# ISAE-PNX/SaDVIO

Hardware: AMD Instinct MI355X
Metric: BA iterations/sec (ms/solve in ms_per_solve), 20-KF/8k-landmark window (higher is better)
Workload: dtype f64; 1 GPU; synthetic 20 KF x 8000 landmarks x 40000 reprojection factors (pixel), GN 10 iters (LM step attempts, early exits disabled); windows_per_gpu=1, parallelism=single window, n_kf=20, n_lmk=8000, n_obs=40000, reduced_dim=114

## Files before the change

sadvio_amd/csrc/ba_handle.h:

```cpp
#pragma once
#include <hip/hip_runtime.h>
#include <dlfcn.h>

#include <algorithm>
#include <chrono>
#include <cmath>
#include <cstdio>
#include <cstdlib>
#include <cstring>
#include <map>
#include <string>
#include <vector>

#include "../../include/sadvio_ba.h"
#include "kernels.h"
#include "layout_plan.h"
#include "dense_chol.h"
#include "marg_kernels.h"
#include "lm_kernels.h"
#include "long_kernels.h"
#include "viinit_kernels.h"
#include "nofov_kernels.h"

using namespace sadvio;
// ... 199 lines not shown
    std::vector<int> h_pairs, h_ptr, h_lmk, h_last;
    int csr_win = -1;
    int n_kf_lmk = 0;
};

struct EnvCfg {
    int debug = 0;
    int lm = -1, pf_wg = -1;
    int tile_rounds = 0, lm_subs = 0, band_c = 0;
    int cov_batch_lds = 1, cov_batch_scratch_mb = 1024;
    int cov_band = -1;
    int cov_sqrt = -1;
    int cov_cross_stage = -1;
    int long_min_env = 0;
    double jacobi_tol = 1e-14;
    bool marg_pivoted = false, marg_unpivoted = false, pchol_strict = false, no_lpt = false, no_pre = false, no_fork = false, no_bcr = false, imu_items = false, contig_tiles = false, c16_old_tail = false;
    void read() {
        auto on = [](const char* k) { return getenv(k) != nullptr; };
        auto num = [](const char* k, int unset) { const char* e = getenv(k); return e ? atoi(e) : unset; };
        debug = num("SADVIO_DEBUG", 0); lm = num("SADVIO_LM", -1); pf_wg = num("SADVIO_PF_WG", -1);
        tile_rounds = num("SADVIO_TILE_ROUNDS", 0); lm_subs = num("SADVIO_LM_SUBS", 0); band_c = num("SADVIO_BAND_C", 0);
        cov_batch_lds = num("SADVIO_COV_BATCH_LDS", 1); cov_batch_scratch_mb = num("SADVIO_COV_BATCH_SCRATCH_MB", 1024);
        cov_band = num("SADVIO_COV_BAND", -1); cov_sqrt = num("SADVIO_COV_SQRT", -1);
        cov_cross_stage = num("SADVIO_COV_CROSS_STAGE", -1);
        long_min_env = num("SADVIO_LONG_MIN", 0);
        if (long_min_env < 2 || long_min_env > MAX_LMK_OBS + 1) long_min_env = 0;
        if (const char* e = getenv("SADVIO_JACOBI_TOL")) jacobi_tol = atof(e);
        marg_pivoted = on("SADVIO_MARG_PIVOTED"); marg_unpivoted = on("SADVIO_MARG_UNPIVOTED"); pchol_strict = on("SADVIO_PCHOL_STRICT");
        no_lpt = on("SADVIO_NO_LPT"); no_pre = on("SADVIO_NO_PRE"); no_fork = on("SADVIO_NO_FORK");
        no_bcr = on("SADVIO_NO_BCR");
        contig_tiles = on("SADVIO_CONTIG_TILES");
        c16_old_tail = on("SADVIO_C16_OLD_TAIL");
        imu_items = on("SADVIO_IMU_ITEMS");
    }
};

struct LongCfg {
    int min = 0;
    bool priors = false;
    bool cov = false;
    bool batch = false;
    bool from_create(unsigned reserved, int long_min_env, std::string& err) {
        static const struct { unsigned flag; const char* name; const char* reason; } needs[] = {
            {SADVIO_CFG_LONG_TRACK_PRIORS, "SADVIO_CFG_LONG_TRACK_PRIORS", "to carry a prior on"},
            {SADVIO_CFG_LONG_TRACK_COVARIANCE, "SADVIO_CFG_LONG_TRACK_COVARIANCE", "to form a covariance of"},
            {SADVIO_CFG_LONG_TRACK_BATCH, "SADVIO_CFG_LONG_TRACK_BATCH", "for a batch call to serve"}};
        for (const auto& n : needs)
// ... 68 lines not shown
    DevBuf<unsigned char> d_lmk_const;
    DevBuf<int> d_lmk_ob, d_lmk_oe, d_obs_kf, d_obs_cam, d_tile_kf, d_tile_row, d_tile_lmk;
    DevBuf<int> d_long_rec, d_long_kf, d_long_slot;
    DevBuf<int> d_pre_lane, d_pre_kf;
    bool pre_dirty = false;
    DevBuf<int> d_rank_col; DevBuf<double> d_rank_x;
    DevBuf<unsigned char> d_obs_slot, d_obs_lslot;
    DevBuf<int> d_chunk_ob, d_chunk_lm, d_tile_perm;
    DevBuf<int> d_jac_ints;
    DevBuf<double> d_jac_dbl;
    DevBuf<double> d_lm_hg, d_lm_dt, d_lm_sacc;
    DevBuf<int> d_lm_sub;
    int hidden_eig_count = 0;
    int marg_stats[4] = {0, 0, 0, 0};
    DevBuf<double> d_ptab;
    DevBuf<double> d_obs_meas;
    DevBuf<PriorDev> d_priors;
    DevBuf<double> d_prior_lin;
    DevBuf<ImuDev> d_imus;
    DevBuf<double> d_imu_scratch;
    DevBuf<double> d_S, d_gred, d_gfull, d_hdiag, d_delta, d_s_pose;
    DevBuf<LmState> d_states;
    DevBuf<double> d_trace;
    DevBuf<long long> d_tstart;
    DevBuf<IterAcc> d_acc;
    DevBuf<FinalRec> d_final;
    FinalRec* h_final = nullptr;
    double* h_deltas = nullptr; size_t h_deltas_cap = 0; bool deltas_cached = false;
    size_t h_final_n = 0;
    std::vector<FinalRec> fin;
// ... 77 lines not shown
```

sadvio_amd/csrc/kernels.h:

```cpp
#pragma once
#include "ba_types.h"
#include "device_math.h"
#include "chol16.h"

namespace sadvio {

struct DevPtrs {
    const WinDev* win;
    const Tile* tiles;
    const double* kf_T0;
    const int* kf_fidx;
    double* xp; double* xv; double* xba; double* xbg;
    long long xp_stride, xv_stride, xl_stride;
    const double* kf_vel; const double* kf_ba; const double* kf_bg;
    const double* cam_K; const double* cam_T; const double* cam_isig;
    const double* lmk_p; double* xl; double* s_lmk;
    const unsigned char* lmk_const;
    const int* lmk_ob; const int* lmk_oe;
    const int* obs_kf; const int* obs_cam; const double* obs_meas;
    const unsigned char* obs_slot;
    const int* tile_kf;
    const int* tile_lmk;
    const int* tile_row;
    const int4* pre_lane;
// ... 36 lines not shown
    double* lm_dt;
    long long lm_hg_stride, lm_dt_stride;
    const int* lm_sub;
    int lm_sub_per_item;
    int lm_ksub;
    double* lm_sacc;
    const LineDev* lines;
    const LineObsDev* lobs;
    double* xline;
    double* line_scratch;
    long long xline_stride;
    long long n_xp, n_xv, n_xl;
    int n_tiles;
    int state_stride;
    int n_win;
    long long* t_start;
    double* trace;
    long long* dbg_ts;
    int debug;
    int c16_old_tail;
    SolveOpts o;
};

#ifdef SADVIO_KERNEL_TS
#define SADVIO_TS(slot_, idx_) do { if ((P.debug & 4096) && blockIdx.x == 0 && threadIdx.x == 0 && slot == (slot_)) P.dbg_ts[idx_] = wall_clock64(); } while (0)
#define SADVIO_TS_PTR(cond_) ((cond_) ? P.dbg_ts : nullptr)
constexpr int DBG_WG_MAX = 1024, DBG_WG_BASE = 128, DBG_SLOTS = DBG_WG_BASE + 4 * DBG_WG_MAX;
#define SADVIO_WG_TS(slot_, which_) do { if ((P.debug & 4096) && blockIdx.x < DBG_WG_MAX && threadIdx.x == 0 && slot == (slot_)) { \
        P.dbg_ts[DBG_WG_BASE + 4 * blockIdx.x + (which_)] = wall_clock64(); \
        if ((which_) == 0) P.dbg_ts[DBG_WG_BASE + 4 * blockIdx.x + 3] = 0; \
        if ((which_) == 0) P.dbg_ts[DBG_WG_BASE + 4 * blockIdx.x + 2] = ((long long)__builtin_amdgcn_s_getreg(20 | (31 << 11)) << 32) | (unsigned)__builtin_amdgcn_s_getreg(4 | (31 << 11)); } } while (0)
#else
#define SADVIO_TS(slot_, idx_) do { } while (0)
#define SADVIO_TS_PTR(cond_) nullptr
#define SADVIO_WG_TS(slot_, which_) do { } while (0)
constexpr int DBG_SLOTS = 128;
// ... 350 lines not shown
        const int lane0 = tid * 8, wv = lane0 >> 6, ln = lane0 & 63;
        const int G = T.G, lpw = 64 / G, grp = ln / G, q0 = ln - grp * G, nl = T.n_lmk;
        const bool valid = wv * lpw + grp < nl;
        const int gl = nl > 0 ? tile_landmark(T, tile_lmk, valid ? wv * lpw + grp : 0) : T.lmk0;
        const int ob = nl > 0 ? lmk_ob[gl] : 0, nobs = (valid && nl > 0) ? lmk_oe[gl] - ob : 0;
        pre_lane[(long long)blockIdx.x * (BUILD_THREADS / 8) + tid] = make_int4(gl, ob, nobs | (valid ? 1 << 16 : 0), q0);
    }
    if (tid < PRE_KF) {
        int2 e = make_int2(-1, -1);
        if (tid < T.n_kf) { e.x = tile_kf[T.kf_off + tid]; e.y = kf_fidx[e.x]; }
        pre_kf[(long long)blockIdx.x * PRE_KF + tid] = e;
    }
}

template <bool COST_ONLY> __device__ __forceinline__ void pose_factor_eval(const DevPtrs& P, int slot, int idx, int ln);
template <int FACTOR, bool RARE, bool IMU>
__global__ __launch_bounds__(BUILD_THREADS, IMU ? 1 : 2) void k_build(DevPtrs P, int slot, int max_tile_kf, int strip_doubles, int Rp) {
    extern __shared__ __attribute__((aligned(16))) char smem[];
    if (IMU && (int)blockIdx.x >= P.n_tiles) {
        pose_factor_eval<false>(P, slot, (int)blockIdx.x - P.n_tiles, threadIdx.x);
        return;
    }
    const Tile T = P.tiles[blockIdx.x];
    const int tid = threadIdx.x, wv = tid >> 6, ln = tid & 63;
    int4 pl = make_int4(0, -1, 0, 0);
    int2 pk = make_int2(-1, -1);
    if (P.pre_lane) {
        pl = P.pre_lane[(long long)blockIdx.x * (BUILD_THREADS / 8) + (tid >> 3)];
        pk = P.pre_kf[(long long)blockIdx.x * PRE_KF + tid / POSE_TAB];
    }
    SADVIO_TS(3, 32);
    SADVIO_WG_TS(3, 0);
    __shared__ double s_part[BUILD_WAVES * 4];
    double* poseTab = (double*)smem;
    double* camTab = poseTab + (size_t)max_tile_kf * POSE_TAB;
    int* rowTab = (int*)(camTab + MAX_WIN_CAM * 17);
    double* stage = (double*)(smem + tile_tables_bytes(max_tile_kf));
// ... 19 lines not shown
            }
        } else {
            const TileAcc* ta = P.tacc + (long long)((slot - 1) & 1) * P.n_tiles + t0;
            double v[4][4];
#pragma unroll
            for (int u = 0; u < 4; u++) {
                const int t = tid + u * BUILD_THREADS;
                const bool in = t < nt;
                const TileAcc* e = ta + (in ? t : 0);
                v[u][0] = in ? e->cand_cost : 0.0; v[u][1] = in ? e->mcc : 0.0; v[u][2] = in ? e->step_norm2 : 0.0; v[u][3] = in ? e->cand_norm2 : 0.0;
            }
            pc = (v[0][0] + v[1][0]) + (v[2][0] + v[3][0]); pm = (v[0][1] + v[1][1]) + (v[2][1] + v[3][1]);
            psn = (v[0][2] + v[1][2]) + (v[2][2] + v[3][2]); pcn = (v[0][3] + v[1][3]) + (v[2][3] + v[3][3]);
        }
    };
    if (P.n_win == 1) decision_inputs(0, 0, P.n_tiles);
    else decision_inputs(T.w, T.win_tile0, T.win_ntiles);
    bool first_valid;
    int gl_first, pre_ob, pre_oe, pre_o;
    static_assert(MAX_LMK_OBS <= 0xff, "a first-round packet carries the landmark's observation count in 8 bits");
    if (P.pre_lane) {
        first_valid = (pl.z >> 16) & 1; gl_first = pl.x; pre_ob = pl.y; pre_oe = pl.y + (pl.z & 0xff);
        pre_o = (pl.w + (tid & 7) < (pl.z & 0xff)) ? pl.y + pl.w + (tid & 7) : -1;
    } else {
        first_valid = wv * lpw + grp < nl;
        gl_first = tile_landmark(T, P.tile_lmk, first_valid ? wv * lpw + grp : 0);
        pre_ob = P.lmk_ob[gl_first]; pre_oe = P.lmk_oe[gl_first];
        pre_o = (first_valid && q < pre_oe - pre_ob) ? pre_ob + q : -1;
    }
    const int pre_lcode = P.lmk_const ? P.lmk_const[gl_first] : 0;
    double pre_p[3], pre_x0[3], pre_x1[3];
#pragma unroll
    for (int i = 0; i < 3; i++) {
        pre_p[i] = P.lmk_p[3 * (long long)gl_first + i];
        pre_x0[i] = P.xl[3 * (long long)gl_first + i];
        pre_x1[i] = P.xl[P.xl_stride + 3 * (long long)gl_first + i];
    }
    double pre_s[3] = {1.0, 1.0, 1.0};
    if (slot != 0) {
#pragma unroll
        for (int i = 0; i < 3; i++) pre_s[i] = P.s_lmk[3 * (long long)gl_first + i];
    }
    double pre_t0 = 0.0, pre_t1 = 0.0;
    if (P.pre_lane) {
        if (pk.x >= 0) {
            const long long src = (long long)pk.x * POSE_TAB + (tid - (tid / POSE_TAB) * POSE_TAB);
            pre_t0 = P.ptab[src]; pre_t1 = P.ptab[P.ptab_stride + src];
        }
    } else if (tid < T.n_kf * POSE_TAB) {
        const int k = tid / POSE_TAB, e = tid - k * POSE_TAB;
        const long long src = (long long)P.tile_kf[T.kf_off + k] * POSE_TAB + e;
        pre_t0 = P.ptab[src]; pre_t1 = P.ptab[P.ptab_stride + src];
    }
    for (int i = tid; i < T.n_cam * 17; i += blockDim.x) {
        const int c = i / 17, e = i - 17 * c;
        const int gc = T.cam_base + c;
        camTab[i] = e < 4 ? P.cam_K[4 * (long long)gc + e] : (e < 16 ? P.cam_T[12 * (long long)gc + e - 4] : P.cam_isig[gc]);
    }
    for (int i = tid; i < T.n_kf; i += blockDim.x) rowTab[i] = P.tile_row[T.kf_off + i];
    ObsPre pre_obs;
    pre_obs.slot = 0; pre_obs.craw = 0; pre_obs.m[0] = pre_obs.m[1] = pre_obs.m[2] = 0.0;
    if (pre_o >= 0) pre_obs = obs_prefetch<FACTOR>(P, pre_o);
    if (own_decision) {
        pc = wave_sum(pc); pm = wave_sum(pm); psn = wave_sum(psn); pcn = wave_sum(pcn);
        if (ln == 0) { s_part[wv * 4] = pc; s_part[wv * 4 + 1] = pm; s_part[wv * 4 + 2] = psn; s_part[wv * 4 + 3] = pcn; }
        __syncthreads();
        a.cand_cost += (s_part[0] + s_part[4]) + (s_part[8] + s_part[12]); a.mcc += (s_part[1] + s_part[5]) + (s_part[9] + s_part[13]);
// ... 1 lines not shown
        st = lm_decide(prev, a, P.o);
        __syncthreads();
        if (T.first_of_window && tid == 0) { P.states[(long long)T.w * P.state_stride + slot] = st; trace_write(P, T.w, slot - 1, prev, a, st); }
    }
    if (st.done) return;
    SADVIO_TS(3, 33);
    double* Stile = stage + BUILD_WAVES * strip_doubles;
    const int Nt = 6 * T.n_free;
    const int tri_n = Nt * (Nt + 1) / 2;
    double* gT = Stile + tri_n;
    double* gfT = gT + Nt;
    double* hdT = gfT + Nt;
    const bool lds_mode = T.lds_mode != 0;
    if (tid < T.n_kf * POSE_TAB) poseTab[tid] = st.cur ? pre_t1 : pre_t0;
    {
        const double* src = P.ptab + (long long)st.cur * P.ptab_stride;
        for (int i = tid + blockDim.x; i < T.n_kf * POSE_TAB; i += blockDim.x) {
            const int k = i / POSE_TAB, e = i - k * POSE_TAB;
            poseTab[i] = src[(long long)P.tile_kf[T.kf_off + k] * POSE_TAB + e];
        }
    }
    if (lds_mode) {
        const int nz = tri_n + 3 * Nt;
        for (int i = tid; i < nz; i += blockDim.x) Stile[i] = 0.0;
    }
    __syncthreads();

    SADVIO_TS(3, 34);
    double* Sg = P.S + T.S_off;
    double* gredg = P.gred + T.red_off;
    double* gfullg = P.gfull + T.red_off;
// ... 18 lines not shown
        if (!first && slot != 0) {
#pragma unroll
            for (int i = 0; i < 3; i++) sc[i] = P.s_lmk[3 * (long long)gl + i];
        }
        ObsLin L;
        L.valid = q < nobs;
        L.row = -1; L.slot = 0; L.counted = false;
        if (L.valid) {
            double pw[3];
            ObsPre obq;
            if (first) {
#pragma unroll
                for (int i = 0; i < 3; i++) pw[i] = pre_p[i] + (st.cur ? pre_x1[i] : pre_x0[i]);
                obq = pre_obs;
            } else {
#pragma unroll
                for (int i = 0; i < 3; i++) pw[i] = P.lmk_p[3 * (long long)gl + i] + xl[3 * (long long)gl + i];
                obq = obs_prefetch<FACTOR>(P, ob + q);
            }
            lane_linearize<FACTOR, RARE>(P, poseTab, camTab, rowTab, T.cam_base, obq, pw, lfree, lcode != 1, L);
            const double c = L.rho;
            if (L.counted) cost_part += c;
            else { fixed_part += c; L.r[0] = 0.0; L.r[1] = 0.0; }
        } else {
            L.r[0] = L.r[1] = 0.0;
#pragma unroll
            for (int i = 0; i < 12; i++) L.Jp[i] = 0.0;
#pragma unroll
            for (int i = 0; i < 6; i++) L.Jl[i] = 0.0;
        }
    SADVIO_TS(3, 35);
        double Mi[6], g[3];
// ... 184 lines not shown
                    const int row = 16 * tr + lk + 4 * rg;
                    if (row < Nt && col <= row) atomic_add_f64(&Stile[tri(row, col)], -accs[pp][rg]);
                }
            }
        }
    }
    SADVIO_TS(3, 40);
    const double c = wave_sum(cost_part), f = wave_sum(fixed_part), gm = wave_max(gmax_part);
    if (ln == 0) { s_part[wv * 4] = c; s_part[wv * 4 + 1] = f; s_part[wv * 4 + 2] = gm; }
    __syncthreads();
    if (tid == 0) {
        double cs = 0.0, fs = 0.0, gs = 0.0;
        for (int k = 0; k < BUILD_WAVES; k++) { cs += s_part[k * 4]; fs += s_part[k * 4 + 1]; gs = fmax(gs, s_part[k * 4 + 2]); }
        TileAcc* ta = P.tacc + (long long)(slot & 1) * P.n_tiles + blockIdx.x;
        ta->lin_cost = cs; ta->fixed_cost = fs; ta->gmax = gs;
    }
    SADVIO_TS(3, 41);
    if (lds_mode) {
        int* growTab = (int*)stage;
        for (int k = tid; k < T.n_kf; k += blockDim.x) {
            const int r = rowTab[k];
            if (r >= 0) {
                const int fi = P.kf_fidx[P.tile_kf[T.kf_off + k]];
#pragma unroll
                for (int i = 0; i < 6; i++) growTab[r + i] = fi * dpf + i;
            }
        }
        __syncthreads();
        if (T.ld) {
            for (int row = wv; row < Nt; row += BUILD_WAVES) {
// ... 1561 lines not shown
}

__device__ __forceinline__ void init_tables_item(const DevPtrs& P, int g, int n_kf_tot) {
    if (g < P.n_prior_tot) {
        const PriorDev pr = P.priors[g];
        double d6[6] = {0.0, 0.0, 0.0, 0.0, 0.0, 0.0};
        prior_lin_record(P.kf_T0 + 12 * (long long)pr.kf, pr.T_prior, pr.inf, d6, P.prior_lin + (long long)g * PRIOR_LIN);
    }
    if (g >= n_kf_tot) return;
    double d6[6], tab[POSE_TAB];
    for (int i = 0; i < 6; i++) d6[i] = 0.0;
    pose_table_entry(P.kf_T0 + 12 * (long long)g, d6, tab);
    for (int i = 0; i < POSE_TAB; i++) P.ptab[(long long)g * POSE_TAB + i] = tab[i];
}

__global__ void k_decide(DevPtrs P, int slot, int final) {
    const int w = blockIdx.x, ln = threadIdx.x;
    __shared__ double s4[4];
    const WinDev W = P.win[w];
    LmState f;
    const bool already = final && P.decide_kernel;
    if (!already) {
        if (P.lm_sacc) {
            __shared__ double sq[16 * 4];
            const long long n = (long long)(W.tile_end - W.tile_begin) * P.lm_ksub;
            const double* sa = P.lm_sacc + ((long long)(slot & 1) * P.n_tiles + W.tile_begin) * P.lm_ksub * 4;
            double c = 0.0, m = 0.0, sn = 0.0, cn = 0.0;
            for (long long t = ln; t < n; t += blockDim.x) { c += sa[4 * t]; m += sa[4 * t + 1]; sn += sa[4 * t + 2]; cn += sa[4 * t + 3]; }
            c = wave_sum(c); m = wave_sum(m); sn = wave_sum(sn); cn = wave_sum(cn);
            if ((ln & 63) == 0) { double* q = sq + 4 * (ln >> 6); q[0] = c; q[1] = m; q[2] = sn; q[3] = cn; }
// ... 663 lines not shown
```

sadvio_amd/csrc/layout_driver.h:

```cpp
#pragma once
#include "ba_handle.h"

namespace {

__global__ void k_dense_prior_prepare(const double* J, double* Jt, int nf, int n) {
    const long long idx = (long long)blockIdx.x * blockDim.x + threadIdx.x;
    if (idx < (long long)nf * n) {
        const int i = (int)(idx / n), a = (int)(idx - (long long)i * n);
        Jt[(size_t)a * nf + i] = J[idx];
    }
}

__global__ void k_sym_from_lower(const double* __restrict__ A, int n, double* __restrict__ H) {
    const long long idx = (long long)blockIdx.x * blockDim.x + threadIdx.x;
    if (idx >= (long long)n * n) return;
    const int i = (int)(idx / n), j = (int)(idx - (long long)i * n);
    H[idx] = i >= j ? A[idx] : A[(size_t)j * n + i];
}

LayoutIn layout_inputs(sadvio_ba_handle* h) {
    LayoutIn in;
    in.src = &h->src; in.sparse_per_win = &h->sparse_per_win; in.dprior_per_win = &h->dprior_per_win; in.lines_per_win = &h->lines_per_win;
    in.prior_valid = h->prior.valid; in.prior_serial = h->prior.serial; in.prior_n_full = h->prior.n_full; in.prior_n = h->prior.n;
    in.world = h->world; in.has_coll = h->coll_fn != nullptr;
// ... 89 lines not shown
        wins[w].d.imu_end = (int)h->imus.size();
    }
    HIP_TRY(h->d_imus.alloc(h->imus.size()));
    HIP_TRY(h->d_imu_scratch.alloc(2 * h->imus.size() * (size_t)IMU_ROW));
    if (!h->imus.empty())
        h->up.add(h->d_imus.p, h->imus.data(), h->imus.size() * sizeof(ImuDev));
    std::vector<WinDev> wd(wins.size());
    for (size_t w = 0; w < wins.size(); w++) wd[w] = wins[w].d;
    h->up.add(h->d_win.p, wd.data(), wd.size() * sizeof(WinDev));
    HIP_TRY(h->up.flush(h->stream));
    if (h->plan.pre_ok && h->pre_dirty) {
        hipLaunchKernelGGL(k_pre_packets, dim3((unsigned)h->plan.tiles.size()), dim3(BUILD_THREADS), 0, h->stream, h->d_tiles.p, h->d_lmk_ob.p, h->d_lmk_oe.p, h->d_tile_kf.p,
                           h->d_tile_lmk.p, h->d_kf_fidx.p, (int4*)h->d_pre_lane.p, (int2*)h->d_pre_kf.p);
        h->pre_dirty = false;
    }
    return SADVIO_OK;
}

int layout_build(sadvio_ba_handle* h) {
    const bool dbg_t = (h->env.debug & 8192) != 0;
    auto t_start = std::chrono::steady_clock::now();
    auto lap = [&](const char* what) { if (dbg_t) { auto t = std::chrono::steady_clock::now(); fprintf(stderr, "[sadvio dbg] build_layout %-14s %.3f ms\n", what, std::chrono::duration<double, std::milli>(t - t_start).count()); t_start = t; } };
    HIP_TRY(hipSetDevice(h->device));
    h->uploaded = false; h->solved = false;
    h->up.reset();
    LayoutPlan& P = h->plan;
    int rc = layout_plan(layout_inputs(h), P, h->err, lap);
    if (rc != SADVIO_OK) return rc;
    const size_t kf_b = P.n_kf_tot, lmk_b = std::max(P.n_lmk_tot, 1), n_tiles = P.tiles.size();
    if (h->env.debug) {
// ... 7 lines not shown
        fprintf(stderr, "\n");
    }
    if (P.want_lm) {
        HIP_TRY(h->d_lm_hg.alloc(2 * (size_t)LM_HG * lmk_b));
        const size_t n_rec = std::max<size_t>(n_tiles, 1) * P.lm_ksub;
        HIP_TRY(h->d_lm_dt.alloc(2 * (size_t)LM_DT * n_rec));
        HIP_TRY(h->d_lm_sacc.alloc(2 * 4 * n_rec));
        HIP_TRY(hipMemsetAsync(h->d_lm_sacc.p, 0, sizeof(double) * 2 * 4 * n_rec, h->stream));
        HIP_TRY(hipMemsetAsync(h->d_lm_dt.p, 0, sizeof(double) * 2 * (size_t)LM_DT * n_rec, h->stream));
    }
    HIP_TRY(h->d_chunk_ob.alloc(P.chunk_ob.size())); HIP_TRY(h->d_chunk_lm.alloc(P.chunk_lm.size())); HIP_TRY(h->d_obs_lslot.alloc(P.obs_lslot.size()));
    HIP_TRY(h->d_tile_perm.alloc(std::max<size_t>(P.perm.size(), 1))); HIP_TRY(h->d_lm_sub.alloc(std::max<size_t>(P.sub.size(), 2)));
    HIP_TRY(h->d_win.alloc(P.wins.size())); HIP_TRY(h->d_tacc.alloc(2 * n_tiles));
    HIP_TRY(h->d_tile_kf.alloc(P.tile_kf.size())); HIP_TRY(h->d_tile_row.alloc(P.tile_row.size())); HIP_TRY(h->d_tile_lmk.alloc(P.tile_lmk.size()));
    HIP_TRY(h->d_obs_slot.alloc(P.obs_slot.size())); HIP_TRY(h->d_ptab.alloc(2 * (size_t)POSE_TAB * kf_b));
    HIP_TRY(h->d_kf_T0.alloc(P.kf_T0.size())); HIP_TRY(h->d_kf_fidx.alloc(P.kf_fidx.size()));
    HIP_TRY(h->d_xp.alloc(2 * 6 * kf_b)); HIP_TRY(h->d_xv.alloc(2 * 3 * kf_b));
    HIP_TRY(h->d_xba.alloc(2 * 3 * kf_b)); HIP_TRY(h->d_xbg.alloc(2 * 3 * kf_b));
    HIP_TRY(h->d_kf_vel.alloc(P.kf_vel.size())); HIP_TRY(h->d_kf_ba.alloc(P.kf_ba.size())); HIP_TRY(h->d_kf_bg.alloc(P.kf_bg.size()));
    HIP_TRY(h->d_cam_K.alloc(P.cam_K.size())); HIP_TRY(h->d_cam_T.alloc(P.cam_T.size())); HIP_TRY(h->d_cam_isig.alloc(P.cam_isig.size()));
    HIP_TRY(h->d_lmk_p.alloc(P.lmk_p.size())); HIP_TRY(h->d_xl.alloc(2 * 3 * lmk_b));
    HIP_TRY(h->d_s_lmk.alloc(3 * lmk_b));
    HIP_TRY(h->d_lmk_ob.alloc(P.lmk_ob.size())); HIP_TRY(h->d_lmk_oe.alloc(P.lmk_oe.size()));
    HIP_TRY(h->d_obs_kf.alloc(P.obs_kf.size())); HIP_TRY(h->d_obs_cam.alloc(P.obs_cam.size())); HIP_TRY(h->d_obs_meas.alloc(P.obs_meas.size()));
    queue_table(h, h->d_chunk_ob, P.chunk_ob); queue_table(h, h->d_chunk_lm, P.chunk_lm); queue_table(h, h->d_obs_lslot, P.obs_lslot);
    queue_table(h, h->d_tile_perm, P.perm); queue_table(h, h->d_lm_sub, P.sub);
    queue_table(h, h->d_kf_T0, P.kf_T0); queue_table(h, h->d_kf_fidx, P.kf_fidx); queue_table(h, h->d_kf_vel, P.kf_vel);
    queue_table(h, h->d_kf_ba, P.kf_ba); queue_table(h, h->d_kf_bg, P.kf_bg); queue_table(h, h->d_cam_K, P.cam_K); queue_table(h, h->d_cam_T, P.cam_T);
    queue_table(h, h->d_cam_isig, P.cam_isig); queue_table(h, h->d_lmk_p, P.lmk_p);
    queue_table(h, h->d_lmk_ob, P.lmk_ob); queue_table(h, h->d_lmk_oe, P.lmk_oe); queue_table(h, h->d_obs_kf, P.obs_kf);
// ... 25 lines not shown
```

sadvio_amd/csrc/solve_driver.h:

```cpp
#pragma once
#include <cstddef>
#include <type_traits>

#include "ba_handle.h"
#include "solve_opts.h"

namespace {

DevPtrs make_ptrs(sadvio_ba_handle* h, const SolveOpts& o, int state_stride) {
    DevPtrs P{};
    P.win = h->d_win.p; P.tiles = h->d_tiles.p;
    P.kf_T0 = h->d_kf_T0.p; P.kf_fidx = h->d_kf_fidx.p;
    P.xp = h->d_xp.p; P.xv = h->d_xv.p; P.xba = h->d_xba.p; P.xbg = h->d_xbg.p;
    P.xp_stride = 6LL * h->plan.n_kf_tot; P.xv_stride = 3LL * h->plan.n_kf_tot; P.xl_stride = 3LL * h->plan.n_lmk_tot;
    P.kf_vel = h->d_kf_vel.p; P.kf_ba = h->d_kf_ba.p; P.kf_bg = h->d_kf_bg.p;
    P.cam_K = h->d_cam_K.p; P.cam_T = h->d_cam_T.p; P.cam_isig = h->d_cam_isig.p;
    P.lmk_p = h->d_lmk_p.p; P.xl = h->d_xl.p; P.s_lmk = h->d_s_lmk.p;
    P.lmk_const = h->plan.has_lmk_const ? h->d_lmk_const.p : nullptr;
    P.lmk_ob = h->d_lmk_ob.p; P.lmk_oe = h->d_lmk_oe.p;
    P.obs_kf = h->d_obs_kf.p; P.obs_cam = h->d_obs_cam.p; P.obs_meas = h->d_obs_meas.p;
    P.obs_slot = h->d_obs_slot.p; P.tile_kf = h->d_tile_kf.p; P.tile_lmk = h->d_tile_lmk.p; P.tile_row = h->d_tile_row.p;
    P.pre_lane = h->plan.pre_ok ? (const int4*)h->d_pre_lane.p : nullptr; P.pre_kf = h->plan.pre_ok ? (const int2*)h->d_pre_kf.p : nullptr;
    P.ptab = h->d_ptab.p; P.ptab_stride = (long long)POSE_TAB * h->plan.n_kf_tot;
    P.priors = h->d_priors.p; P.prior_lin = h->d_prior_lin.p; P.prior_lin_stride = (long long)h->priors.size() * PRIOR_LIN; P.n_prior_tot = (int)h->priors.size();
    P.imus = h->d_imus.p; P.imu_scratch = h->d_imu_scratch.p; P.imu_scratch_stride = (long long)h->imus.size() * IMU_ROW;
    P.S = h->d_S.p; P.gred = h->d_gred.p; P.gfull = h->d_gfull.p; P.hdiag = h->d_hdiag.p;
    P.delta = h->d_delta.p; P.s_pose = h->d_s_pose.p;
    P.dbg_ts = h->d_dbg.p;
    P.trace = h->d_trace.p; P.t_start = h->d_tstart.p;
    P.states = h->d_states.p; P.acc = h->d_acc.p; P.tacc = h->d_tacc.p; P.n_tiles = (int)h->plan.tiles.size();
    P.state_stride = state_stride;
    P.final_out = h->h_final ? h->h_final : h->d_final.p;
    P.big_info = h->d_big_info.p;
    P.world = h->world; P.rank = h->rank; P.rank_b = h->d_rank_b.p; P.rank_s = h->d_rank_s.p;
    P.lmk_red = h->d_lmk_red.p; P.kept_obs = h->d_kept_obs.p; P.n_kept = h->plan.n_kept;
    P.dp_data = h->d_dp_data.p; P.dp_ints = h->d_dp_ints.p;
    P.sparse = h->d_sparse.p; P.sp_scratch = h->d_sp_scratch.p; P.sp_list = h->d_sp_list.p;
// ... 72 lines not shown
    }
};

#define SADVIO_TILE_VARIANTS(K) {{{K<1, false, false>, K<1, false, true>}, {K<1, true, false>, K<1, true, true>}}, \
                                 {{K<0, false, false>, K<0, false, true>}, {K<0, true, false>, K<0, true, true>}}}
using BuildFn = decltype(&k_build<0, false, false>);
using BacksubFn = decltype(&k_backsub<0, false, false>);
BuildFn build_variant(bool pix, bool rare, bool with_imu) {
    static const BuildFn t[2][2][2] = SADVIO_TILE_VARIANTS(k_build);
    return t[pix][rare][with_imu];
}
BacksubFn backsub_variant(bool pix, bool rare, bool with_imu) {
    static const BacksubFn t[2][2][2] = SADVIO_TILE_VARIANTS(k_backsub);
    return t[pix][rare][with_imu];
}
#undef SADVIO_TILE_VARIANTS

struct SolvePlan {
    DevPtrs P;
    int slots;
    int mtk, Rp, strip_doubles;
    int n_kf_tot, n_pf, n_lo, dp_max_nf, dp_max_n, reset_blocks, table_blocks, max_win_tiles, lm_n_sub, lm_sub_obs, n_big;
    bool pix, rare, with_imu, use_lm, extras, fork;
    bool coll_band;
    size_t lds_build, lds_back, lds_solve, lds_bobs, lds_pass0, lds_pass, lds_long_lin, lds_long_back;
    BuildFn k_build;
    BacksubFn k_backsub;
    decltype(&k_build_kept<0>) k_build_kept;
    decltype(&k_build_obs<0>) k_build_obs;
    LongArgs lg;
    decltype(&k_long_lin<0>) k_long_lin;
    decltype(&k_long_back<0>) k_long_back;
    decltype(&k_lm_pass<0, false>) k_lm_pass, k_lm_pass0;
    decltype(&k_solve<0, false>) k_solve, k_solve_front, k_solve_back;
    double *big_linv, *big_mid, *big_M, *big_Lx, *bcr;
    double* coll_buf;
    long long coll_count;
};
static_assert(std::is_trivially_copyable<SolvePlan>::value && std::is_trivially_copyable<BigPlan>::value, "the graph key is their bytes");

size_t band_lds_bytes(int R, int nb, int blocks) {
// ... 195 lines not shown
    for (int w = 0; w < n_win; w++) {
        const WinDev& d = h->plan.wins[w].d;
        if (d.imu_end > d.imu_begin || d.sp_end > d.sp_begin || d.dp_n_full > 0 || d.dpf == 15 || d.lobs_end > d.lobs_begin || d.line_end > d.line_begin) extras = true;
    }
    plan.extras = extras;
    plan.k_solve = extras ? k_solve<0, true> : k_solve<0, false>;
    plan.k_solve_front = extras ? k_solve<1, true> : k_solve<1, false>;
    plan.k_solve_back = extras ? k_solve<2, true> : k_solve<2, false>;
    HIP_TRY(hipFuncSetAttribute((const void*)plan.k_solve, hipFuncAttributeMaxDynamicSharedMemorySize, (int)plan.lds_solve));
    plan.n_kf_tot = h->plan.n_kf_tot; plan.n_big = h->plan.n_big;
    plan.reset_blocks = (int)std::min<long long>(1024, std::max<long long>(1, (P.n_xl + P.n_xp + 255) / 256));
    plan.table_blocks = (std::max(h->plan.n_kf_tot, (int)h->priors.size()) + 63) / 64;
    plan.n_pf = (int)h->imus.size() + h->n_sp_list;
    plan.n_lo = h->n_lobs_tot;
    plan.fork = plan.n_lo > 0 && h->side && !h->cfg.profile_kernels && !h->coll_fn && !h->env.no_fork;
    big.clear(); big.resize(n_win);
    if (n_win) memset(big.data(), 0, sizeof(BigPlan) * (size_t)n_win);
    for (int w = 0; w < n_win; w++) {
        const WinDev& d = h->plan.wins[w].d;
        if (!d.ld) continue;
        BigPlan& p = big[w];
        p.Np = d.Np; p.ld = d.ld; p.dpf = d.dpf; p.red_off = d.red_off; p.S_off = d.S_off;
        p.bw = window_bandwidth(h, w);
    }
    if (h->coll_fn && h->world > 1 && h->plan.n_big) {
        std::vector<double> slots((size_t)n_win * h->world * 4, 0.0);
        for (int w = 0; w < n_win; w++) slots[((size_t)w * h->world + h->rank) * 4] = (double)big[w].bw;
        HIP_TRY(hipMemcpyAsync(h->d_rank_s.p, slots.data(), slots.size() * sizeof(double), hipMemcpyHostToDevice, h->stream));
        if (h->coll_fn(h->coll_ctx, h->d_rank_s.p, (int64_t)slots.size(), (void*)h->stream) != 0) { h->err = "solve: all-reduce failed"; return SADVIO_E_RCCL; }
        HIP_TRY(hipMemcpyAsync(slots.data(), h->d_rank_s.p, slots.size() * sizeof(double), hipMemcpyDeviceToHost, h->stream));
// ... 27 lines not shown
        if (n_win == 1 && big[0].ld && big[0].bw < big[0].Np && big[0].S_off == 0) {
            const long long nbd = (long long)big[0].Np * big[0].bw, tail = h->plan.red_total - (long long)big[0].Np * big[0].ld;
            HIP_TRY(h->d_coll_band.alloc((size_t)(nbd + tail)));
            plan.coll_band = true; plan.coll_buf = h->d_coll_band.p; plan.coll_count = nbd + tail;
        }
    }
    for (int w = 0; w < n_win; w++) { plan.dp_max_nf = std::max(plan.dp_max_nf, h->plan.wins[w].d.dp_n_full); plan.dp_max_n = std::max(plan.dp_max_n, h->plan.wins[w].d.dp_n); }
    return SADVIO_OK;
}

bool enqueue_solve(sadvio_ba_handle* h, const SolvePlan& pl, const std::vector<BigPlan>& big) {
    const DevPtrs& P = pl.P;
    const int n_win = P.n_win, n_tiles = P.n_tiles, n_kept = P.n_kept, mtk = pl.mtk, n_pf = pl.n_pf, n_lo = pl.n_lo;
    const bool fork = pl.fork, use_lm = pl.use_lm, with_imu = pl.with_imu;
    bool coll_ok = true;
    {
        ScopedTimer t(h, "k_reset");
        hipLaunchKernelGGL(k_reset, dim3(pl.reset_blocks + pl.table_blocks), dim3(256), 0, h->stream, P, pl.reset_blocks, pl.n_kf_tot);
    }
    for (int s = 0; s < pl.slots; s++) {
        if (fork) {
            (void)hipEventRecord(h->ev_fork, h->stream);
            (void)hipStreamWaitEvent(h->side, h->ev_fork, 0);
            if (n_lo) hipLaunchKernelGGL(k_line_eval<true>, dim3(n_lo), dim3(64), 0, h->side, P, s, 1);
            (void)hipEventRecord(h->ev_lin, h->side);
        }
        if (use_lm) {
            if (s == 0) { ScopedTimer t(h, "k_lm_pass0"); hipLaunchKernelGGL(pl.k_lm_pass0, dim3(pl.lm_n_sub), dim3(LM_PASS_THREADS), pl.lds_pass0, h->stream, P, s, mtk, pl.lm_sub_obs); }
            { ScopedTimer t(h, "k_build_obs"); hipLaunchKernelGGL(pl.k_build_obs, dim3(n_tiles), dim3(BUILD_THREADS), pl.lds_bobs, h->stream, P, s, mtk, pl.Rp); }
        } else
        { ScopedTimer t(h, "k_build"); hipLaunchKernelGGL(pl.k_build, dim3(n_tiles + (with_imu ? n_pf : 0)), dim3(BUILD_THREADS), pl.lds_build, h->stream, P, s, mtk, pl.strip_doubles, pl.Rp); }
        if (n_pf && (use_lm || !with_imu)) { ScopedTimer t(h, "k_pf_lin"); hipLaunchKernelGGL(k_pf_eval<false>, dim3(n_pf), dim3(BUILD_THREADS), 0, h->stream, P, s); }
        if (n_kept) { ScopedTimer t(h, "k_build_kept"); hipLaunchKernelGGL(pl.k_build_kept, dim3((n_kept + 127) / 128), dim3(128), 0, h->stream, P, s); }
        if (pl.lg.n_long) { ScopedTimer t(h, "k_long_lin"); hipLaunchKernelGGL(pl.k_long_lin, dim3(pl.lg.n_long), dim3(LONG_THREADS), pl.lds_long_lin, h->stream, P, pl.lg, s); }
        if (pl.dp_max_nf > 0) {
            ScopedTimer t(h, "k_prior_r+gh");
            const int colb = (pl.dp_max_n + 3) / 4;
            hipLaunchKernelGGL(k_prior_r, dim3((pl.dp_max_nf + 3) / 4, n_win), dim3(256), 0, h->stream, P, s);
            hipLaunchKernelGGL(k_prior_gh, dim3(colb + (unsigned)(((long long)pl.dp_max_n * pl.dp_max_n + 255) / 256), n_win), dim3(256), 0, h->stream, P, s, colb);
        }
        if (h->coll_fn) {
            { ScopedTimer t(h, "k_rank_partials"); hipLaunchKernelGGL(k_rank_partials, dim3(n_win), dim3(64), 0, h->stream, P, s, 0); }
            ScopedTimer t(h, "allreduce_reduced_system");
            if (pl.coll_band) {
                const BigPlan& b0 = big[0];
                const long long nbd = (long long)b0.Np * b0.bw, tail = pl.coll_count - nbd;
// ... 210 lines not shown
```

Measured before the change: 19470 BA iterations/s.

## Fold the reset kernel into the first build launch via rider workgroups

Removes the separate k_reset launch on the plain pixel path by adding extra workgroups to the slot-0 k_build launch that zero state buffers, reset LM states and init tables. The slot-0 build tiles no longer read state written by the reset: they use a precomputed zero-delta pose table (ptab0), skip reading xl, and construct the initial LmState themselves. The intent is to cut one kernel launch and its serialization from each solve. It relies on the build tiles not depending on what the riders write, and it adds a template variant plus a one-time ptab0 precompute.

```diff
diff --git a/sadvio_amd/csrc/ba_handle.h b/sadvio_amd/csrc/ba_handle.h
--- a/sadvio_amd/csrc/ba_handle.h
+++ b/sadvio_amd/csrc/ba_handle.h
@@ -237,7 +237,7 @@
     int cov_cross_stage = -1;
     int long_min_env = 0;
     double jacobi_tol = 1e-14;
-    bool marg_pivoted = false, marg_unpivoted = false, pchol_strict = false, no_lpt = false, no_pre = false, no_fork = false, no_bcr = false, imu_items = false, contig_tiles = false, c16_old_tail = false;
+    bool marg_pivoted = false, marg_unpivoted = false, pchol_strict = false, no_lpt = false, no_pre = false, no_fork = false, no_bcr = false, imu_items = false, contig_tiles = false, c16_old_tail = false, reset_kernel = false;
     void read() {
         auto on = [](const char* k) { return getenv(k) != nullptr; };
         auto num = [](const char* k, int unset) { const char* e = getenv(k); return e ? atoi(e) : unset; };
@@ -254,6 +254,7 @@
         no_bcr = on("SADVIO_NO_BCR");
         contig_tiles = on("SADVIO_CONTIG_TILES");
         c16_old_tail = on("SADVIO_C16_OLD_TAIL");
+        reset_kernel = on("SADVIO_RESET_KERNEL");
         imu_items = on("SADVIO_IMU_ITEMS");
     }
 };
@@ -352,6 +353,8 @@
     int hidden_eig_count = 0;
     int marg_stats[4] = {0, 0, 0, 0};
     DevBuf<double> d_ptab;
+    DevBuf<double> d_ptab0;
+    bool ptab0_dirty = false;
     DevBuf<double> d_obs_meas;
     DevBuf<PriorDev> d_priors;
     DevBuf<double> d_prior_lin;
diff --git a/sadvio_amd/csrc/kernels.h b/sadvio_amd/csrc/kernels.h
--- a/sadvio_amd/csrc/kernels.h
+++ b/sadvio_amd/csrc/kernels.h
@@ -74,12 +74,14 @@
     int n_tiles;
     int state_stride;
     int n_win;
+    int reset_ride;
     long long* t_start;
     double* trace;
     long long* dbg_ts;
     int debug;
     int c16_old_tail;
     SolveOpts o;
+    const double* ptab0;
 };
 
 #ifdef SADVIO_KERNEL_TS
@@ -460,13 +462,20 @@
 }
 
 template <bool COST_ONLY> __device__ __forceinline__ void pose_factor_eval(const DevPtrs& P, int slot, int idx, int ln);
-template <int FACTOR, bool RARE, bool IMU>
+__device__ __forceinline__ void reset_ride_wg(const DevPtrs& P, int rider);
+template <int FACTOR, bool RARE, bool IMU, bool RIDE = false>
 __global__ __launch_bounds__(BUILD_THREADS, IMU ? 1 : 2) void k_build(DevPtrs P, int slot, int max_tile_kf, int strip_doubles, int Rp) {
     extern __shared__ __attribute__((aligned(16))) char smem[];
     if (IMU && (int)blockIdx.x >= P.n_tiles) {
         pose_factor_eval<false>(P, slot, (int)blockIdx.x - P.n_tiles, threadIdx.x);
         return;
     }
+    static_assert(!(RIDE && IMU), "the IMU pairs' workgroups read what the riders write");
+    if (RIDE && (int)blockIdx.x >= P.n_tiles) {
+        reset_ride_wg(P, (int)blockIdx.x - P.n_tiles);
+        return;
+    }
+    constexpr bool ride0 = RIDE;
     const Tile T = P.tiles[blockIdx.x];
     const int tid = threadIdx.x, wv = tid >> 6, ln = tid & 63;
     int4 pl = make_int4(0, -1, 0, 0);
@@ -516,7 +525,11 @@
             psn = (v[0][2] + v[1][2]) + (v[2][2] + v[3][2]); pcn = (v[0][3] + v[1][3]) + (v[2][3] + v[3][3]);
         }
     };
-    if (P.n_win == 1) decision_inputs(0, 0, P.n_tiles);
+    if (ride0) {
+        st = LmState{};
+        st.radius = P.o.initial_radius; st.decrease_factor = 2.0;
+    }
+    else if (P.n_win == 1) decision_inputs(0, 0, P.n_tiles);
     else decision_inputs(T.w, T.win_tile0, T.win_ntiles);
     bool first_valid;
     int gl_first, pre_ob, pre_oe, pre_o;
@@ -531,12 +544,15 @@
         pre_o = (first_valid && q < pre_oe - pre_ob) ? pre_ob + q : -1;
     }
     const int pre_lcode = P.lmk_const ? P.lmk_const[gl_first] : 0;
-    double pre_p[3], pre_x0[3], pre_x1[3];
-#pragma unroll
-    for (int i = 0; i < 3; i++) {
-        pre_p[i] = P.lmk_p[3 * (long long)gl_first + i];
-        pre_x0[i] = P.xl[3 * (long long)gl_first + i];
-        pre_x1[i] = P.xl[P.xl_stride + 3 * (long long)gl_first + i];
+    double pre_p[3], pre_x0[3] = {0.0, 0.0, 0.0}, pre_x1[3] = {0.0, 0.0, 0.0};
+#pragma unroll
+    for (int i = 0; i < 3; i++) pre_p[i] = P.lmk_p[3 * (long long)gl_first + i];
+    if (!ride0) {
+#pragma unroll
+        for (int i = 0; i < 3; i++) {
+            pre_x0[i] = P.xl[3 * (long long)gl_first + i];
+            pre_x1[i] = P.xl[P.xl_stride + 3 * (long long)gl_first + i];
+        }
     }
     double pre_s[3] = {1.0, 1.0, 1.0};
     if (slot != 0) {
@@ -544,15 +560,16 @@
         for (int i = 0; i < 3; i++) pre_s[i] = P.s_lmk[3 * (long long)gl_first + i];
     }
     double pre_t0 = 0.0, pre_t1 = 0.0;
+    const double* tab0 = ride0 ? P.ptab0 : P.ptab;
     if (P.pre_lane) {
         if (pk.x >= 0) {
             const long long src = (long long)pk.x * POSE_TAB + (tid - (tid / POSE_TAB) * POSE_TAB);
-            pre_t0 = P.ptab[src]; pre_t1 = P.ptab[P.ptab_stride + src];
+            pre_t0 = tab0[src]; pre_t1 = P.ptab[P.ptab_stride + src];
         }
     } else if (tid < T.n_kf * POSE_TAB) {
         const int k = tid / POSE_TAB, e = tid - k * POSE_TAB;
         const long long src = (long long)P.tile_kf[T.kf_off + k] * POSE_TAB + e;
-        pre_t0 = P.ptab[src]; pre_t1 = P.ptab[P.ptab_stride + src];
+        pre_t0 = tab0[src]; pre_t1 = P.ptab[P.ptab_stride + src];
     }
     for (int i = tid; i < T.n_cam * 17; i += blockDim.x) {
         const int c = i / 17, e = i - 17 * c;
@@ -584,7 +601,7 @@
     const bool lds_mode = T.lds_mode != 0;
     if (tid < T.n_kf * POSE_TAB) poseTab[tid] = st.cur ? pre_t1 : pre_t0;
     {
-        const double* src = P.ptab + (long long)st.cur * P.ptab_stride;
+        const double* src = ride0 ? P.ptab0 : P.ptab + (long long)st.cur * P.ptab_stride;
         for (int i = tid + blockDim.x; i < T.n_kf * POSE_TAB; i += blockDim.x) {
             const int k = i / POSE_TAB, e = i - k * POSE_TAB;
             poseTab[i] = src[(long long)P.tile_kf[T.kf_off + k] * POSE_TAB + e];
@@ -633,8 +650,13 @@
                 for (int i = 0; i < 3; i++) pw[i] = pre_p[i] + (st.cur ? pre_x1[i] : pre_x0[i]);
                 obq = pre_obs;
             } else {
-#pragma unroll
-                for (int i = 0; i < 3; i++) pw[i] = P.lmk_p[3 * (long long)gl + i] + xl[3 * (long long)gl + i];
+                double xq[3] = {0.0, 0.0, 0.0};
+                if (!ride0) {
+#pragma unroll
+                    for (int i = 0; i < 3; i++) xq[i] = xl[3 * (long long)gl + i];
+                }
+#pragma unroll
+                for (int i = 0; i < 3; i++) pw[i] = P.lmk_p[3 * (long long)gl + i] + xq[i];
                 obq = obs_prefetch<FACTOR>(P, ob + q);
             }
             lane_linearize<FACTOR, RARE>(P, poseTab, camTab, rowTab, T.cam_base, obq, pw, lfree, lcode != 1, L);
@@ -849,6 +871,7 @@
         for (int k = 0; k < BUILD_WAVES; k++) { cs += s_part[k * 4]; fs += s_part[k * 4 + 1]; gs = fmax(gs, s_part[k * 4 + 2]); }
         TileAcc* ta = P.tacc + (long long)(slot & 1) * P.n_tiles + blockIdx.x;
         ta->lin_cost = cs; ta->fixed_cost = fs; ta->gmax = gs;
+        if (ride0) { ta->cand_cost = 0.0; ta->mcc = 0.0; ta->step_norm2 = 0.0; ta->cand_norm2 = 0.0; ta->pad = 0.0; }
     }
     SADVIO_TS(3, 41);
     if (lds_mode) {
@@ -2440,6 +2463,43 @@
     for (int i = 0; i < POSE_TAB; i++) P.ptab[(long long)g * POSE_TAB + i] = tab[i];
 }
 
+__device__ __forceinline__ void ride_zero(double* p, long long n, long long t, long long nt) {
+    double2* p2 = (double2*)p;
+    const double2 z2 = make_double2(0.0, 0.0);
+    for (long long i = t; i < (n >> 1); i += nt) p2[i] = z2;
+    if ((n & 1) && t == 0) p[n - 1] = 0.0;
+}
+__device__ __forceinline__ void reset_ride_wg(const DevPtrs& P, int rider) {
+    const long long t = (long long)rider * blockDim.x + threadIdx.x, nt = (long long)P.reset_ride * blockDim.x;
+    if (t == 0 && P.t_start) *P.t_start = wall_clock64();
+    ride_zero(P.xp, P.n_xp, t, nt);
+    ride_zero(P.xv, P.n_xv, t, nt); ride_zero(P.xba, P.n_xv, t, nt); ride_zero(P.xbg, P.n_xv, t, nt);
+    ride_zero(P.xl, P.n_xl, t, nt);
+    ride_zero(P.xline, 2 * P.xline_stride, t, nt);
+    static_assert(sizeof(IterAcc) % 8 == 0 && sizeof(TileAcc) % 16 == 0, "ride_zero writes doubles, 16 bytes at a time");
+    ride_zero((double*)P.acc, (long long)P.n_win * P.state_stride * (long long)(sizeof(IterAcc) / 8), t, nt);
+    ride_zero((double*)(P.tacc + P.n_tiles), (long long)P.n_tiles * (long long)(sizeof(TileAcc) / 8), t, nt);
+    const long long ns = (long long)P.n_win * P.state_stride;
+    if (P.trace) ride_zero(P.trace, ns * 8, t, nt);
+    for (long long i = t; i < ns; i += nt) {
+        LmState z{};
+        if (i % P.state_stride == 0) { z.radius = P.o.initial_radius; z.decrease_factor = 2.0; }
+        P.states[i] = z;
+    }
+    const int n_kf_tot = (int)(P.ptab_stride / POSE_TAB);
+    const int n_items = n_kf_tot > P.n_prior_tot ? n_kf_tot : P.n_prior_tot;
+    for (long long g = t; g < n_items; g += nt) init_tables_item(P, (int)g, n_kf_tot);
+}
+
+__global__ __launch_bounds__(64) void k_ptab0(const double* __restrict__ kf_T0, double* __restrict__ ptab0, int n_kf_tot) {
+    const int g = (int)blockIdx.x * 64 + threadIdx.x;
+    if (g >= n_kf_tot) return;
+    double d6[6], tab[POSE_TAB];
+    for (int i = 0; i < 6; i++) d6[i] = 0.0;
+    pose_table_entry(kf_T0 + 12 * (long long)g, d6, tab);
+    for (int i = 0; i < POSE_TAB; i++) ptab0[(long long)g * POSE_TAB + i] = tab[i];
+}
+
 __global__ void k_decide(DevPtrs P, int slot, int final) {
     const int w = blockIdx.x, ln = threadIdx.x;
     __shared__ double s4[4];
diff --git a/sadvio_amd/csrc/layout_driver.h b/sadvio_amd/csrc/layout_driver.h
--- a/sadvio_amd/csrc/layout_driver.h
+++ b/sadvio_amd/csrc/layout_driver.h
@@ -127,6 +127,10 @@
                            h->d_tile_lmk.p, h->d_kf_fidx.p, (int4*)h->d_pre_lane.p, (int2*)h->d_pre_kf.p);
         h->pre_dirty = false;
     }
+    if (h->ptab0_dirty && h->plan.n_kf_tot > 0) {
+        hipLaunchKernelGGL(k_ptab0, dim3((unsigned)((h->plan.n_kf_tot + 63) / 64)), dim3(64), 0, h->stream, h->d_kf_T0.p, h->d_ptab0.p, h->plan.n_kf_tot);
+        h->ptab0_dirty = false;
+    }
     return SADVIO_OK;
 }
 
@@ -164,6 +168,7 @@
     HIP_TRY(h->d_win.alloc(P.wins.size())); HIP_TRY(h->d_tacc.alloc(2 * n_tiles));
     HIP_TRY(h->d_tile_kf.alloc(P.tile_kf.size())); HIP_TRY(h->d_tile_row.alloc(P.tile_row.size())); HIP_TRY(h->d_tile_lmk.alloc(P.tile_lmk.size()));
     HIP_TRY(h->d_obs_slot.alloc(P.obs_slot.size())); HIP_TRY(h->d_ptab.alloc(2 * (size_t)POSE_TAB * kf_b));
+    HIP_TRY(h->d_ptab0.alloc((size_t)POSE_TAB * kf_b)); h->ptab0_dirty = true;
     HIP_TRY(h->d_kf_T0.alloc(P.kf_T0.size())); HIP_TRY(h->d_kf_fidx.alloc(P.kf_fidx.size()));
     HIP_TRY(h->d_xp.alloc(2 * 6 * kf_b)); HIP_TRY(h->d_xv.alloc(2 * 3 * kf_b));
     HIP_TRY(h->d_xba.alloc(2 * 3 * kf_b)); HIP_TRY(h->d_xbg.alloc(2 * 3 * kf_b));
diff --git a/sadvio_amd/csrc/solve_driver.h b/sadvio_amd/csrc/solve_driver.h
--- a/sadvio_amd/csrc/solve_driver.h
+++ b/sadvio_amd/csrc/solve_driver.h
@@ -21,6 +21,7 @@
     P.obs_kf = h->d_obs_kf.p; P.obs_cam = h->d_obs_cam.p; P.obs_meas = h->d_obs_meas.p;
     P.obs_slot = h->d_obs_slot.p; P.tile_kf = h->d_tile_kf.p; P.tile_lmk = h->d_tile_lmk.p; P.tile_row = h->d_tile_row.p;
     P.pre_lane = h->plan.pre_ok ? (const int4*)h->d_pre_lane.p : nullptr; P.pre_kf = h->plan.pre_ok ? (const int2*)h->d_pre_kf.p : nullptr;
+    P.ptab0 = h->d_ptab0.p;
     P.ptab = h->d_ptab.p; P.ptab_stride = (long long)POSE_TAB * h->plan.n_kf_tot;
     P.priors = h->d_priors.p; P.prior_lin = h->d_prior_lin.p; P.prior_lin_stride = (long long)h->priors.size() * PRIOR_LIN; P.n_prior_tot = (int)h->priors.size();
     P.imus = h->d_imus.p; P.imu_scratch = h->d_imu_scratch.p; P.imu_scratch_stride = (long long)h->imus.size() * IMU_ROW;
@@ -123,6 +124,10 @@
     static const BacksubFn t[2][2][2] = SADVIO_TILE_VARIANTS(k_backsub);
     return t[pix][rare][with_imu];
 }
+BuildFn build_ride_variant(bool pix, bool rare) {
+    static const BuildFn t[2][2] = {{k_build<1, false, false, true>, k_build<1, true, false, true>}, {k_build<0, false, false, true>, k_build<0, true, false, true>}};
+    return t[pix][rare];
+}
 #undef SADVIO_TILE_VARIANTS
 
 struct SolvePlan {
@@ -131,9 +136,11 @@
     int mtk, Rp, strip_doubles;
     int n_kf_tot, n_pf, n_lo, dp_max_nf, dp_max_n, reset_blocks, table_blocks, max_win_tiles, lm_n_sub, lm_sub_obs, n_big;
     bool pix, rare, with_imu, use_lm, extras, fork;
+    int ride;
     bool coll_band;
     size_t lds_build, lds_back, lds_solve, lds_bobs, lds_pass0, lds_pass, lds_long_lin, lds_long_back;
     BuildFn k_build;
+    BuildFn k_build0;
     BacksubFn k_backsub;
     decltype(&k_build_kept<0>) k_build_kept;
     decltype(&k_build_obs<0>) k_build_obs;
@@ -359,6 +366,15 @@
     plan.n_pf = (int)h->imus.size() + h->n_sp_list;
     plan.n_lo = h->n_lobs_tot;
     plan.fork = plan.n_lo > 0 && h->side && !h->cfg.profile_kernels && !h->coll_fn && !h->env.no_fork;
+    if (!use_lm && !with_imu && !plan.fork && plan.n_lo == 0 && P.world == 1 && !h->coll_fn && !P.decide_kernel && n_tiles > 0 &&
+        n_tiles <= PRE_MAX_TILES && !h->env.reset_kernel) {
+        const long long bytes = 8 * (P.n_xp + 3 * P.n_xv + P.n_xl + 2 * P.xline_stride) + (long long)n_win * stride * (long long)(sizeof(IterAcc) + 64 + sizeof(LmState)) +
+                                (long long)n_tiles * (long long)sizeof(TileAcc);
+        plan.ride = (int)std::min<long long>(16, std::max<long long>(1, (bytes + 32767) / 32768));
+    }
+    P.reset_ride = plan.ride;
+    plan.k_build0 = plan.ride ? build_ride_variant(pix, rare) : plan.k_build;
+    HIP_TRY(hipFuncSetAttribute((const void*)plan.k_build0, hipFuncAttributeMaxDynamicSharedMemorySize, (int)plan.lds_build));
     big.clear(); big.resize(n_win);
     if (n_win) memset(big.data(), 0, sizeof(BigPlan) * (size_t)n_win);
     for (int w = 0; w < n_win; w++) {
@@ -416,7 +432,7 @@
     const int n_win = P.n_win, n_tiles = P.n_tiles, n_kept = P.n_kept, mtk = pl.mtk, n_pf = pl.n_pf, n_lo = pl.n_lo;
     const bool fork = pl.fork, use_lm = pl.use_lm, with_imu = pl.with_imu;
     bool coll_ok = true;
-    {
+    if (!pl.ride) {
         ScopedTimer t(h, "k_reset");
         hipLaunchKernelGGL(k_reset, dim3(pl.reset_blocks + pl.table_blocks), dim3(256), 0, h->stream, P, pl.reset_blocks, pl.n_kf_tot);
     }
@@ -431,7 +447,7 @@
             if (s == 0) { ScopedTimer t(h, "k_lm_pass0"); hipLaunchKernelGGL(pl.k_lm_pass0, dim3(pl.lm_n_sub), dim3(LM_PASS_THREADS), pl.lds_pass0, h->stream, P, s, mtk, pl.lm_sub_obs); }
             { ScopedTimer t(h, "k_build_obs"); hipLaunchKernelGGL(pl.k_build_obs, dim3(n_tiles), dim3(BUILD_THREADS), pl.lds_bobs, h->stream, P, s, mtk, pl.Rp); }
         } else
-        { ScopedTimer t(h, "k_build"); hipLaunchKernelGGL(pl.k_build, dim3(n_tiles + (with_imu ? n_pf : 0)), dim3(BUILD_THREADS), pl.lds_build, h->stream, P, s, mtk, pl.strip_doubles, pl.Rp); }
+        { ScopedTimer t(h, "k_build"); hipLaunchKernelGGL(s == 0 ? pl.k_build0 : pl.k_build, dim3(n_tiles + (with_imu ? n_pf : 0) + (s == 0 ? pl.ride : 0)), dim3(BUILD_THREADS), pl.lds_build, h->stream, P, s, mtk, pl.strip_doubles, pl.Rp); }
         if (n_pf && (use_lm || !with_imu)) { ScopedTimer t(h, "k_pf_lin"); hipLaunchKernelGGL(k_pf_eval<false>, dim3(n_pf), dim3(BUILD_THREADS), 0, h->stream, P, s); }
         if (n_kept) { ScopedTimer t(h, "k_build_kept"); hipLaunchKernelGGL(pl.k_build_kept, dim3((n_kept + 127) / 128), dim3(128), 0, h->stream, P, s); }
         if (pl.lg.n_long) { ScopedTimer t(h, "k_long_lin"); hipLaunchKernelGGL(pl.k_long_lin, dim3(pl.lg.n_long), dim3(LONG_THREADS), pl.lds_long_lin, h->stream, P, pl.lg, s); }
```

Result: no change. 19610 BA iterations/s, median of 6 (+0.7%).
